# ValentinoGuerrini/Configurable-Hierarchical-Allreduce-Algorithms

Hardware: AMD Instinct MI355X
Metric: device-resident bucket-reduction GB/s (fp32); allreduce GB/s at 2/4/8 GPUs (higher is better)
Workload: dtype f32; 1 GPU; C2 bucket reduction: k=2 (m=1 incoming bucket), 64 MiB fp32 per bucket, device-resident, MPI_Reduce_local semantics; bucket_bytes=67108864, m=1, buffer_sets=16, parallelism=replicas, gate=untimed spin kernel ahead of the start event

## Files before the change

### include/chiara_user_op.hpp

```cpp
#pragma once

#include <hip/hip_runtime.h>

#include <cstddef>
#include <cstdint>
#include <type_traits>

#include "chiara.h"

namespace chr_user {

constexpr int kMaxIns = 16;
#ifndef CHR_USER_FOLD_U
#define CHR_USER_FOLD_U 4
#endif
constexpr int kU = CHR_USER_FOLD_U;

struct FoldArgs {
    void* out;
    const void* acc;
    const void* ins[kMaxIns];
    int m;
    size_t n;
    int running_first;
    int vec;
};

template <typename T>
struct FoldVec {
    static constexpr int kN = (sizeof(T) <= 16 && 16 % sizeof(T) == 0) ? int(16 / sizeof(T)) : 1;
    T e[kN];
};

typedef unsigned int tree_w4 __attribute__((ext_vector_type(4)));
typedef unsigned int tree_w2 __attribute__((ext_vector_type(2)));

#ifndef CHR_USER_GROUP_VEC
#define CHR_USER_GROUP_VEC 1
#endif
constexpr bool group_fold_pays(size_t s) { return s == 48; }
constexpr bool group_tree_pays(size_t s) { return s == 32; }
constexpr size_t gcd16(size_t s) {
    size_t g = 16;
    while (s % g) g >>= 1;
    return g;
}
template <typename T>
struct Grp {
    static constexpr size_t S = sizeof(T), G = S / gcd16(S) * 16;
    static constexpr int V = int(G / 16), E = int(G / S), kHeads = int(16 / gcd16(S));
    static constexpr bool kWide = 16 % S != 0;
    static constexpr bool kCan = kWide && V <= 8;
    static constexpr bool kFold = kCan && (CHR_USER_GROUP_VEC == 2 || (CHR_USER_GROUP_VEC == 1 && group_fold_pays(S)));
    static constexpr bool kTree =
        kCan && S % 4 == 0 && (CHR_USER_GROUP_VEC == 2 || (CHR_USER_GROUP_VEC == 1 && group_tree_pays(S)));
    static constexpr int kFoldU = !kFold ? 0 : 8 / V < kU ? 8 / V : kU;
};
template <int V> struct GrpW { tree_w4 w[V]; };
template <typename T> struct GrpE { T e[Grp<T>::E]; };
template <typename T> struct GrpPad { T t; unsigned char pad[(sizeof(T) + 3) / 4 * 4 - sizeof(T)]; };
template <typename T, typename OP>
__device__ __forceinline__ GrpW<Grp<T>::V> grp_map(const GrpW<Grp<T>::V>& a, const GrpW<Grp<T>::V>& b, OP op) {
    constexpr int V = Grp<T>::V, E = Grp<T>::E;
    using W = GrpW<V>;
    if constexpr (sizeof(T) % 4 == 0) {
        const GrpE<T> ae = __builtin_bit_cast(GrpE<T>, a), be = __builtin_bit_cast(GrpE<T>, b);
        GrpE<T> re;
#pragma unroll
        for (int e = 0; e < E; ++e) re.e[e] = op(ae.e[e], be.e[e]);
        return __builtin_bit_cast(W, re);
    } else {
        constexpr int S = (int)sizeof(T), NT = (S + 3) / 4, NW = 4 * V;
        struct Words { uint32_t w[NW]; };
        struct Elem { uint32_t w[NT]; };
        const Words aw = __builtin_bit_cast(Words, a), bw = __builtin_bit_cast(Words, b);
        Words rw = {};
        auto get = [](const Words& g, int o) {
            Elem t;
#pragma unroll
            for (int k = 0; k < NT; ++k) {
                const int q = o / 4 + k, sh = o % 4 * 8;
                uint32_t lo = g.w[q];
                if (sh) lo = (lo >> sh) | (q + 1 < NW ? g.w[q + 1] << (32 - sh) : 0u);
                t.w[k] = lo;
            }
            return __builtin_bit_cast(GrpPad<T>, t).t;
        };
#pragma unroll
        for (int e = 0; e < E; ++e) {
            GrpPad<T> p = {};
            p.t = op(get(aw, e * S), get(bw, e * S));
            const Elem t = __builtin_bit_cast(Elem, p);
#pragma unroll
            for (int k = 0; k < NT; ++k) {
                const int nb = S - 4 * k < 4 ? S - 4 * k : 4, o = e * S + 4 * k, q = o / 4, sh = o % 4 * 8;
                const uint32_t v = nb == 4 ? t.w[k] : t.w[k] & ((1u << (8 * nb)) - 1u);
                rw.w[q] |= v << sh;
                if (sh && sh + 8 * nb > 32) rw.w[q + 1] |= v >> (32 - sh);
            }
        }
        return __builtin_bit_cast(W, rw);
    }
}

inline bool congruent16(const void* p, const void* q) { return (((uintptr_t)p ^ (uintptr_t)q) & 15) == 0; }
template <typename T>
inline int group_head(const void* p, size_t n) {
    for (int h = 0; h < Grp<T>::kHeads; ++h)
        if ((((uintptr_t)p + (uintptr_t)h * sizeof(T)) & 15) == 0) return (size_t)h <= n ? h : -1;
    return -1;
}

template <typename T, typename F>
__device__ __forceinline__ void fold_groups(const FoldArgs& a) {
    constexpr int V = Grp<T>::V, E = Grp<T>::E, U = Grp<T>::kFoldU;
    using W = GrpW<V>;
    const F f{};
    const size_t tid = (size_t)blockIdx.x * blockDim.x + threadIdx.x;
    const size_t stride = (size_t)gridDim.x * blockDim.x;
    const size_t h = (size_t)a.vec - 1, ngrp = (a.n - h) / E, off = h * sizeof(T);
    const bool rf = a.running_first != 0;
    const W* accg = reinterpret_cast<const W*>(static_cast<const char*>(a.acc) + off);
    W* outg = reinterpret_cast<W*>(static_cast<char*>(a.out) + off);
    auto one = [&](T r, T x) { return f(rf ? r : x, rf ? x : r); };
    auto comb = [&](W& r, const W& x) { r = grp_map<T>(r, x, one); };
    const size_t chunk = (size_t)U * blockDim.x;
    const size_t nfull = ngrp / chunk;
    for (size_t c = blockIdx.x; c < nfull; c += gridDim.x) {
        const size_t base = c * chunk + threadIdx.x;
        W r[U];
#pragma unroll
        for (int u = 0; u < U; ++u) r[u] = accg[base + (size_t)u * blockDim.x];
        for (int j = 0; j < a.m; ++j) {
            const W* ing = reinterpret_cast<const W*>(static_cast<const char*>(a.ins[j]) + off);
            W x[U];
#pragma unroll
            for (int u = 0; u < U; ++u) x[u] = ing[base + (size_t)u * blockDim.x];
#pragma unroll
            for (int u = 0; u < U; ++u) comb(r[u], x[u]);
        }
#pragma unroll
        for (int u = 0; u < U; ++u) outg[base + (size_t)u * blockDim.x] = r[u];
    }
    for (size_t g = nfull * chunk + tid; g < ngrp; g += stride) {
        W r = accg[g];
        for (int j = 0; j < a.m; ++j)
            comb(r, reinterpret_cast<const W*>(static_cast<const char*>(a.ins[j]) + off)[g]);
        outg[g] = r;
    }
    const size_t tail0 = h + ngrp * E, extra = h + (a.n - tail0);
    for (size_t t = tid; t < extra; t += stride) {
        const size_t i = t < h ? t : tail0 + (t - h);
        T r = static_cast<const T*>(a.acc)[i];
        for (int j = 0; j < a.m; ++j) r = one(r, static_cast<const T*>(a.ins[j])[i]);
        static_cast<T*>(a.out)[i] = r;
    }
}

template <typename T, typename F>
__global__ void k_fold(FoldArgs a) {
    using V = FoldVec<T>;
    constexpr int kN = V::kN;
    const F f{};
    const size_t tid = (size_t)blockIdx.x * blockDim.x + threadIdx.x;
    const size_t stride = (size_t)gridDim.x * blockDim.x;
    if constexpr (Grp<T>::kFold) {
        if (a.vec) {
            fold_groups<T, F>(a);
            return;
        }
    }
    size_t done = 0;
    if (kN > 1 && a.vec) {
        const size_t nv = a.n / kN;
        const V* accv = static_cast<const V*>(a.acc);
        V* outv = static_cast<V*>(a.out);
        const size_t chunk = (size_t)kU * blockDim.x;
        const size_t nfull = nv / chunk;
        for (size_t c = blockIdx.x; c < nfull; c += gridDim.x) {
            const size_t base = c * chunk + threadIdx.x;
            V r[kU];
#pragma unroll
            for (int u = 0; u < kU; ++u) r[u] = accv[base + (size_t)u * blockDim.x];
            for (int j = 0; j < a.m; ++j) {
                const V* inv = static_cast<const V*>(a.ins[j]);
                V x[kU];
#pragma unroll
                for (int u = 0; u < kU; ++u) x[u] = inv[base + (size_t)u * blockDim.x];
#pragma unroll
                for (int u = 0; u < kU; ++u)
#pragma unroll
                    for (int e = 0; e < kN; ++e)
                        r[u].e[e] = a.running_first ? f(r[u].e[e], x[u].e[e]) : f(x[u].e[e], r[u].e[e]);
            }
#pragma unroll
            for (int u = 0; u < kU; ++u) outv[base + (size_t)u * blockDim.x] = r[u];
        }
        for (size_t v = nfull * chunk + tid; v < nv; v += stride) {
            V r = accv[v];
            for (int j = 0; j < a.m; ++j) {
                const V x = static_cast<const V*>(a.ins[j])[v];
#pragma unroll
                for (int e = 0; e < kN; ++e) r.e[e] = a.running_first ? f(r.e[e], x.e[e]) : f(x.e[e], r.e[e]);
            }
            outv[v] = r;
        }
        done = nv * kN;
    }
    for (size_t i = done + tid; i < a.n; i += stride) {
        T r = static_cast<const T*>(a.acc)[i];
        for (int j = 0; j < a.m; ++j) {
            const T x = static_cast<const T*>(a.ins[j])[i];
            r = a.running_first ? f(r, x) : f(x, r);
        }
        static_cast<T*>(a.out)[i] = r;
    }
}

template <typename T, typename F>
int launch_fold(void* out, const void* acc, const void* const* ins, int m, size_t n, int running_first,
                hipStream_t stream) {
    if (m < 0) return 1;
    const unsigned block = 256;
    auto aligned = [](const void* p) { return ((uintptr_t)p & 15) == 0; };
    bool vec = aligned(out) && aligned(acc);
    for (int j = 0; j < m; ++j) vec = vec && aligned(ins[j]);
    size_t lanes = vec ? (n / FoldVec<T>::kN + kU - 1) / kU + n % FoldVec<T>::kN : n;
    int head = -1;
    if constexpr (Grp<T>::kFold) {
        bool same = congruent16(out, acc);
        for (int j = 0; j < m; ++j) same = same && congruent16(out, ins[j]);
        if (same) head = group_head<T>(out, n);
        if (head >= 0)
            lanes = ((n - head) / Grp<T>::E + Grp<T>::kFoldU - 1) / Grp<T>::kFoldU + Grp<T>::kHeads + Grp<T>::E;
        else
            lanes = n;
    }
    const size_t blocks = (lanes + block - 1) / block;
    const unsigned grid = (unsigned)(blocks < 4096 ? (blocks ? blocks : 1) : 4096);
    int done = 0;
    const void* cur = acc;
    do {
        FoldArgs a{};
        a.out = out;
        a.acc = cur;
        a.m = m - done < kMaxIns ? m - done : kMaxIns;
        for (int j = 0; j < a.m; ++j) a.ins[j] = ins[done + j];
        a.n = n;
        a.running_first = running_first;
        a.vec = Grp<T>::kFold ? head + 1 : vec ? 1 : 0;
        hipLaunchKernelGGL((k_fold<T, F>), dim3(grid), dim3(block), 0, stream, a);
        if (hipGetLastError() != hipSuccess) return 1;
        done += a.m;
        cur = out;
    } while (done < m);
    return 0;
}

constexpr int kMaxLeaves = 8;
constexpr int kMaxTreesPerLaunch = 8;
constexpr int kTreeBlock = 64;
constexpr size_t kMaxLeafBytes = (size_t)1 << 37;
constexpr uint32_t kMaxElementwiseBlocks = 4096;

template <int NL>
constexpr int tree_u() {
    return NL <= 2 ? 4 : NL <= 4 ? 2 : 1;
}
template <typename T, int NL>
constexpr int tree_u_for() {
    if (!Grp<T>::kWide) return tree_u<NL>();
    if (!Grp<T>::kTree) return 0;
    return 8 / (NL * Grp<T>::V) < tree_u<NL>() ? 8 / (NL * Grp<T>::V) : tree_u<NL>();
}
#ifndef CHR_USER_TREE_WIDE_ELEMENTWISE
#define CHR_USER_TREE_WIDE_ELEMENTWISE 1
#endif
#ifndef CHR_USER_TREE_WG_PER_CU
#define CHR_USER_TREE_WG_PER_CU(NL) ((NL) <= 4 ? 12 : 16)
#endif

#ifndef CHR_USER_TREE_NT
#define CHR_USER_TREE_NT 1
#endif
#ifndef CHR_USER_TREE_XCD_RUN_KIB
#define CHR_USER_TREE_XCD_RUN_KIB 256
#endif

__device__ __forceinline__ tree_w4 tree_ld(const tree_w4* p) {
#if CHR_USER_TREE_NT
    return __builtin_nontemporal_load(p);
#else
    return *p;
#endif
}
__device__ __forceinline__ void tree_st(tree_w4* p, tree_w4 v) {
#if CHR_USER_TREE_NT
    __builtin_nontemporal_store(v, p);
#else
    *p = v;
#endif
}

template <int TRIP_BYTES>
__device__ __forceinline__ uint32_t tree_trip(uint32_t lb, uint32_t nblk) {
    constexpr uint32_t R = (uint32_t)CHR_USER_TREE_XCD_RUN_KIB * 1024u / TRIP_BYTES;
    if constexpr (R > 1) {
        constexpr uint32_t span = 8 * R;
        if (lb < nblk / span * span) {
            const uint32_t w = lb % span;
            return lb - w + (w % 8) * R + w / 8;
        }
    }
    return lb;
}

struct TreeSeg {
    void* out;
    const void* leaves[kMaxLeaves];
    size_t n;
    uint32_t comb;
    uint32_t swaps;
    uint32_t vec;
    uint32_t nblk;
};
struct TreeArgs {
    uint32_t block0[kMaxTreesPerLaunch];
    TreeSeg seg[kMaxTreesPerLaunch];
};

template <typename T, bool ARITH = std::is_arithmetic<T>::value, size_t SZ = sizeof(T)>
struct TreeSlot { using S = T; };
template <typename T> struct TreeSlot<T, false, 4> { using S = uint32_t; };
template <typename T> struct TreeSlot<T, false, 8> { using S = tree_w2; };
template <typename T> struct TreeSlot<T, false, 16> { using S = tree_w4; };

template <typename T, typename F>
struct TreeApVec {
    using S = tree_w4;
    __device__ __forceinline__ static S ap(S in, S run) {
        using V = FoldVec<T>;
        const V x = __builtin_bit_cast(V, in);
        V r = __builtin_bit_cast(V, run);
        const F f{};
#pragma unroll
        for (int e = 0; e < V::kN; ++e) r.e[e] = f(x.e[e], r.e[e]);
        return __builtin_bit_cast(S, r);
    }
};
template <typename T, typename F>
struct TreeApGrp {
    using S = GrpW<Grp<T>::V>;
    __device__ __forceinline__ static S ap(const S& in, const S& run) {
        return grp_map<T>(in, run, [](const T& x, const T& r) { return F{}(x, r); });
    }
};
template <typename T, typename F>
struct TreeApOne {
    using S = typename TreeSlot<T>::S;
    __device__ __forceinline__ static S ap(S in, S run) {
        return __builtin_bit_cast(S, F{}(__builtin_bit_cast(T, in), __builtin_bit_cast(T, run)));
    }
};

template <typename A, int NL, int W, bool WIDE = false>
__device__ __forceinline__ void tree_eval(const typename A::S (&x)[NL][W], typename A::S (&r)[W], uint32_t comb,
                                          uint32_t swaps) {
    using S = typename A::S;
#pragma unroll
    for (int w = 0; w < W; ++w) {
        S s0 = x[0][w], s1 = s0, s2 = s0, s3 = s0;
        int d = 1, ci = 0;
#pragma unroll
        for (int j = 1; j < NL; ++j) {
            const S v = x[j][w];
            if constexpr (WIDE) {
                if (d == 1) s1 = v;
                else if (j > 1 && d == 2) s2 = v;
                else if (j > 2) s3 = v;
            } else {
                if (d == 1) s1 = v;
                else if (d == 2) s2 = v;
                else s3 = v;
            }
            ++d;
            for (int c = (int)((comb >> (2 * j)) & 3u); c > 0; --c, ++ci) {
                const bool sw = (swaps >> ci) & 1u;
                if constexpr (WIDE) {
                    if (j == 1 || d == 2) {
                        if (sw) s0 = A::ap(s0, s1);
                        else s0 = A::ap(s1, s0);
                    } else if (j == 2 || d == 3) {
                        if (sw) s1 = A::ap(s1, s2);
                        else s1 = A::ap(s2, s1);
                    } else {
                        if (sw) s2 = A::ap(s2, s3);
                        else s2 = A::ap(s3, s2);
                    }
                } else {
                    if (d == 2) s0 = A::ap(sw ? s0 : s1, sw ? s1 : s0);
                    else if (d == 3) s1 = A::ap(sw ? s1 : s2, sw ? s2 : s1);
                    else s2 = A::ap(sw ? s2 : s3, sw ? s3 : s2);
                }
                --d;
            }
        }
        r[w] = s0;
    }
}

template <typename T, typename F, int NL>
__device__ __forceinline__ void tree_one(const TreeSeg& g, size_t i) {
    using A = TreeApOne<T, F>;
    using S = typename A::S;
    S x[NL][1], r[1];
#pragma unroll
    for (int j = 0; j < NL; ++j) x[j][0] = __builtin_bit_cast(S, static_cast<const T*>(g.leaves[j])[i]);
    tree_eval<A, NL, 1, Grp<T>::kWide>(x, r, g.comb, g.swaps);
    static_cast<T*>(g.out)[i] = __builtin_bit_cast(T, r[0]);
}

template <typename T, typename F, int NL, int U, int BL>
__global__ __launch_bounds__(BL) void k_tree(TreeArgs a) {
    using V = FoldVec<T>;
    constexpr int kN = V::kN;
    const uint32_t b = blockIdx.x;
    int s = 0;
#pragma unroll
    for (int j = 1; j < kMaxTreesPerLaunch; ++j)
        if (b >= a.block0[j]) s = j;
    const TreeSeg& g = a.seg[s];
    const uint32_t nblk = g.nblk;
    if (b - a.block0[s] >= nblk) return;
    constexpr int kTripBytes = U == 0 ? BL * (int)sizeof(T) : BL * U * 16 * (Grp<T>::kWide ? Grp<T>::V : 1);
    const uint32_t lb = tree_trip<kTripBytes>(b - a.block0[s], nblk);
    const size_t n = g.n;
    if constexpr (Grp<T>::kTree && U > 0) if (g.vec) {
        using A = TreeApGrp<T, F>;
        using W = typename A::S;
        constexpr int E = Grp<T>::E;
        const size_t h = g.vec - 1, ngrp = (n - h) / E, nfull = ngrp / ((size_t)BL * U), off = h * sizeof(T);
        const uint32_t comb = g.comb, swaps = g.swaps;
        W* const out = reinterpret_cast<W*>(static_cast<char*>(g.out) + off);
        const W* lv[NL];
#pragma unroll
        for (int j = 0; j < NL; ++j) lv[j] = reinterpret_cast<const W*>(static_cast<const char*>(g.leaves[j]) + off);
        if (lb < nfull) {
            const size_t base = (size_t)lb * BL * U + threadIdx.x;
            W x[NL][U], r[U];
#pragma unroll
            for (int j = 0; j < NL; ++j)
#pragma unroll
                for (int u = 0; u < U; ++u)
#pragma unroll
                    for (int v = 0; v < Grp<T>::V; ++v) x[j][u].w[v] = tree_ld(&lv[j][base + (size_t)u * BL].w[v]);
            __builtin_amdgcn_sched_barrier(0);
            tree_eval<A, NL, U, true>(x, r, comb, swaps);
#pragma unroll
            for (int u = 0; u < U; ++u)
#pragma unroll
                for (int v = 0; v < Grp<T>::V; ++v) tree_st(&out[base + (size_t)u * BL].w[v], r[u].w[v]);
        }
        if (lb == nfull) {
            for (size_t i = nfull * BL * U + threadIdx.x; i < ngrp; i += BL) {
                W x[NL][1], r[1];
#pragma unroll
                for (int j = 0; j < NL; ++j) x[j][0] = lv[j][i];
                tree_eval<A, NL, 1, true>(x, r, comb, swaps);
                out[i] = r[0];
            }
        }
        if (lb == 0) {
            const size_t tail0 = h + ngrp * E, t = threadIdx.x;
            const size_t i = t < h ? t : tail0 + (t - h);
            if (i < n) tree_one<T, F, NL>(g, i);
        }
        return;
    }
    if constexpr (sizeof(V) == 16) if (g.vec) {
        using A = TreeApVec<T, F>;
        const size_t nvec = n / kN, nfull = nvec / ((size_t)BL * U);
        const uint32_t comb = g.comb, swaps = g.swaps;
        tree_w4* const out = static_cast<tree_w4*>(g.out);
        const tree_w4* lv[NL];
#pragma unroll
        for (int j = 0; j < NL; ++j) lv[j] = static_cast<const tree_w4*>(g.leaves[j]);
        if (lb < nfull) {
            const size_t base = (size_t)lb * BL * U + threadIdx.x;
            tree_w4 x[NL][U], r[U];
#pragma unroll
            for (int j = 0; j < NL; ++j)
#pragma unroll
                for (int u = 0; u < U; ++u) x[j][u] = tree_ld(&lv[j][base + (size_t)u * BL]);
            __builtin_amdgcn_sched_barrier(0);
            tree_eval<A, NL, U>(x, r, comb, swaps);
#pragma unroll
            for (int u = 0; u < U; ++u) tree_st(&out[base + (size_t)u * BL], r[u]);
        }
        if (lb == nfull) {
            for (size_t i = nfull * BL * U + threadIdx.x; i < nvec; i += BL) {
                tree_w4 x[NL][1], r[1];
#pragma unroll
                for (int j = 0; j < NL; ++j) x[j][0] = lv[j][i];
                tree_eval<A, NL, 1>(x, r, comb, swaps);
                out[i] = r[0];
            }
        }
        if (lb == 0 && nvec * kN + threadIdx.x < n) tree_one<T, F, NL>(g, nvec * kN + threadIdx.x);
        return;
    }
    for (size_t i = (size_t)lb * BL + threadIdx.x; i < n; i += (size_t)nblk * BL) tree_one<T, F, NL>(g, i);
}

inline unsigned tree_lds_bytes(int wg_per_cu) {
    static const struct Lds {
        int cu = 0, blk = 0;
        Lds() {
            int dev = 0;
            if (hipGetDevice(&dev) != hipSuccess ||
                hipDeviceGetAttribute(&cu, hipDeviceAttributeMaxSharedMemoryPerMultiprocessor, dev) != hipSuccess ||
                hipDeviceGetAttribute(&blk, hipDeviceAttributeMaxSharedMemoryPerBlock, dev) != hipSuccess)
                cu = blk = 0;
        }
    } lds;
    if (wg_per_cu <= 0 || lds.cu <= 0 || lds.blk <= 0) return 0;
    const unsigned bytes = ((unsigned)lds.cu / (unsigned)wg_per_cu) & ~255u;
    return bytes > (unsigned)lds.blk ? (unsigned)lds.blk & ~255u : bytes;
}

template <typename T, typename F, int NL>
void launch_tree_nl(const chr_user_tree* const* trees, int ntrees, int wg_per_cu, hipStream_t stream) {
    constexpr int U = tree_u_for<T, NL>(), BL = kTreeBlock;
    constexpr bool kVecT = sizeof(FoldVec<T>) == 16;
    constexpr bool kGrpT = Grp<T>::kTree && U > 0;
    static_assert(!kGrpT || Grp<T>::kHeads + Grp<T>::E <= BL, "head and tail elements: one lane each");
    const unsigned lds = tree_lds_bytes(wg_per_cu > 0 ? wg_per_cu : CHR_USER_TREE_WG_PER_CU(NL));
    auto aligned = [](const void* p) { return ((uintptr_t)p & 15) == 0; };
    for (int t0 = 0; t0 < ntrees; t0 += kMaxTreesPerLaunch) {
        TreeArgs a{};
        uint32_t grid = 0;
        for (int k = 0; k < kMaxTreesPerLaunch; ++k) {
            if (t0 + k >= ntrees) {
                a.block0[k] = ~0u;
                continue;
            }
            const chr_user_tree& t = *trees[t0 + k];
            TreeSeg& g = a.seg[k];
            g.out = t.out;
            bool vec = kVecT && aligned(t.out);
            int ci = 0;
            for (int j = 0; j < NL; ++j) {
                g.leaves[j] = t.leaves[j];
                vec = vec && aligned(t.leaves[j]);
                g.comb |= (uint32_t)(t.comb[j] & 3u) << (2 * j);
                for (int c = 0; c < t.comb[j] && ci < 8; ++c, ++ci) g.swaps |= (uint32_t)(t.swaps[ci] & 1u) << ci;
            }
            g.n = t.n;
            g.vec = vec ? 1 : 0;
            const size_t per = vec ? (size_t)BL * U * FoldVec<T>::kN : (size_t)BL;
            size_t want = (t.n + per - 1) / per;
            if constexpr (kGrpT) {
                bool same = true;
                for (int j = 0; j < NL; ++j) same = same && congruent16(t.out, t.leaves[j]);
                const int head = same ? group_head<T>(t.out, t.n) : -1;
                if (head >= 0) {
                    vec = true;
                    g.vec = 1u + (uint32_t)head;
                    const size_t ngrp = (t.n - head) / Grp<T>::E, trip = (size_t)BL * U;
                    want = ngrp < trip ? 1 : (ngrp + trip - 1) / trip;
                }
            }
            g.nblk = (uint32_t)(vec || want < kMaxElementwiseBlocks ? want : kMaxElementwiseBlocks);
            a.block0[k] = grid;
            grid += (g.nblk + 7u) & ~7u;
        }
        hipLaunchKernelGGL((k_tree<T, F, NL, U, BL>), dim3(grid), dim3(BL), lds, stream, a);
    }
}

template <typename T, typename F>
int launch_tree(const chr_user_tree* trees, int ntrees, int wg_per_cu, hipStream_t stream) {
    if (ntrees < 0 || (ntrees && !trees)) return 1;
    for (int t = 0; t < ntrees; ++t) {
        const chr_user_tree& tr = trees[t];
        if (tr.nleaves < 2 || tr.nleaves > kMaxLeaves || tr.n == 0 || tr.n > kMaxLeafBytes / sizeof(T) ||
            !tr.out)
            return 1;
        int d = 0;
        for (int j = 0; j < tr.nleaves; ++j) {
            if (!tr.leaves[j] || ++d > 4 || tr.comb[j] > 3 || tr.comb[j] >= d) return 1;
            d -= tr.comb[j];
        }
        if (d != 1) return 1;
        if (Grp<T>::kTree && !CHR_USER_TREE_WIDE_ELEMENTWISE && tr.nleaves * Grp<T>::V > 8) return 1;
    }
    const chr_user_tree* grp[64];
    for (int nl = 2; nl <= kMaxLeaves; ++nl) {
        int k = 0;
        auto flush = [&] {
            if (k == 0) return;
            switch (nl) {
            case 2: launch_tree_nl<T, F, 2>(grp, k, wg_per_cu, stream); break;
            case 3: launch_tree_nl<T, F, 3>(grp, k, wg_per_cu, stream); break;
            case 4: launch_tree_nl<T, F, 4>(grp, k, wg_per_cu, stream); break;
            case 5: launch_tree_nl<T, F, 5>(grp, k, wg_per_cu, stream); break;
            case 6: launch_tree_nl<T, F, 6>(grp, k, wg_per_cu, stream); break;
            case 7: launch_tree_nl<T, F, 7>(grp, k, wg_per_cu, stream); break;
            default: launch_tree_nl<T, F, 8>(grp, k, wg_per_cu, stream); break;
            }
            k = 0;
        };
        for (int t = 0; t < ntrees; ++t)
            if (trees[t].nleaves == nl) {
                grp[k++] = &trees[t];
                if (k == 64) flush();
            }
        flush();
    }
    return 0;
}

}

#define CHR_DEFINE_USER_TREE(name, T, F)                                                                             \
    extern "C" int name(const chr_user_tree* trees, int ntrees, chr_dtype, int wg_per_cu, hipStream_t stream,        \
                        void*) {                                                                                     \
        return chr_user::launch_tree<T, F>(trees, ntrees, wg_per_cu, stream);                                        \
    }

#define CHR_DEFINE_USER_TREE_FOR(name, T, F, DTYPE)                                                                   \
    extern "C" int name(const chr_user_tree* trees, int ntrees, chr_dtype dt, int wg_per_cu, hipStream_t stream,     \
                        void*) {                                                                                     \
        if (dt != (DTYPE)) return 1;                                                                                 \
        return chr_user::launch_tree<T, F>(trees, ntrees, wg_per_cu, stream);                                        \
    }

#define CHR_DEFINE_USER_OP(name, T, F)                                                                               \
    extern "C" int name(void* out, const void* acc, const void* const* ins, int m, size_t n, chr_dtype,             \
                        int running_first, hipStream_t stream, void*) {                                           \
        return chr_user::launch_fold<T, F>(out, acc, ins, m, n, running_first, stream);                           \
    }

#define CHR_DEFINE_USER_OP_FOR(name, T, F, DTYPE)                                                                     \
    extern "C" int name(void* out, const void* acc, const void* const* ins, int m, size_t n, chr_dtype dt,          \
                        int running_first, hipStream_t stream, void*) {                                           \
        if (dt != (DTYPE)) return 1;                                                                                 \
        return chr_user::launch_fold<T, F>(out, acc, ins, m, n, running_first, stream);                           \
    }
```

Measured before the change: 6744 GB/s.

## Add streaming fold kernel with XCD-aware block mapping for large buckets

Adds a specialized streaming path for the fold (reduce_local) kernel on large, aligned, non-wide types. Each 64-thread block handles a fixed tile with U-way unroll and nontemporal loads and stores. Block indices are remapped so consecutive runs of memory stay on one XCD, kernel arguments are pinned to SGPRs, and LDS is reserved to cap workgroups per CU. The tree path also gets a plain (cached) first load and an optional SGPR pin. The aim is to get closer to HBM streaming bandwidth for the 64 MiB m=1 case, at the cost of extra template instantiations and a size-threshold dispatch.

```diff
diff --git a/include/chiara_user_op.hpp b/include/chiara_user_op.hpp
--- a/include/chiara_user_op.hpp
+++ b/include/chiara_user_op.hpp
@@ -24,6 +24,7 @@
     size_t n;
     int running_first;
     int vec;
+    int stream;
 };
 
 template <typename T>
@@ -157,10 +158,119 @@
     }
 }
 
+#ifndef CHR_USER_FOLD_STREAM_MIN_BYTES
+#define CHR_USER_FOLD_STREAM_MIN_BYTES ((size_t)40 << 20)
+#endif
+constexpr int kMaxStreamIns = 8;
+constexpr int kStreamBlock = 64;
+constexpr int kStreamWgPerCu = 12;
+constexpr int stream_u(int m) { return m == 1 ? 4 : m <= 3 ? 2 : 1; }
+constexpr int stream_run_kib(int m) { return m <= 3 ? 256 : 512; }
+
+template <typename P>
+__device__ __forceinline__ void pin_sgpr(P p) {
+    asm volatile("" ::"s"(p));
+}
+
+template <int TRIP_BYTES, int RUN_KIB>
+__device__ __forceinline__ uint32_t xcd_run_trip(uint32_t lb, uint32_t nblk) {
+    constexpr uint32_t R = (uint32_t)RUN_KIB * 1024u / TRIP_BYTES;
+    if constexpr (R > 1) {
+        constexpr uint32_t span = 8 * R;
+        if (lb < nblk / span * span) {
+            const uint32_t w = lb % span;
+            return lb - w + (w % 8) * R + w / 8;
+        }
+    }
+    return lb;
+}
+
+inline unsigned tree_lds_bytes(int wg_per_cu);
+
+template <typename T, typename F, int M>
+__device__ __forceinline__ void fold_stream(const FoldArgs& a) {
+    using V = FoldVec<T>;
+    constexpr int kN = V::kN, U = stream_u(M), BL = kStreamBlock;
+    static_assert(sizeof(V) == 16 && kN <= BL, "FoldVec's sizes only");
+    const F f{};
+    tree_w4* const out = static_cast<tree_w4*>(a.out);
+    const tree_w4* const accp = static_cast<const tree_w4*>(a.acc);
+    const tree_w4* ins[M];
+#pragma unroll
+    for (int j = 0; j < M; ++j) ins[j] = static_cast<const tree_w4*>(a.ins[j]);
+    const size_t n = a.n;
+    const int rf = a.running_first;
+    pin_sgpr(out);
+    pin_sgpr(accp);
+    pin_sgpr(n);
+    pin_sgpr(rf);
+#pragma unroll
+    for (int j = 0; j < M; ++j) pin_sgpr(ins[j]);
+    const size_t nv = n / kN, nfull = nv / ((size_t)BL * U);
+    const size_t lb = xcd_run_trip<BL * U * 16, stream_run_kib(M)>(blockIdx.x, gridDim.x);
+    auto comb = [&](tree_w4& r, tree_w4 x) {
+        const V p = __builtin_bit_cast(V, rf ? r : x), q = __builtin_bit_cast(V, rf ? x : r);
+        V o;
+#pragma unroll
+        for (int e = 0; e < kN; ++e) o.e[e] = f(p.e[e], q.e[e]);
+        r = __builtin_bit_cast(tree_w4, o);
+    };
+    if (lb < nfull) {
+        const size_t base = lb * BL * U + threadIdx.x;
+        tree_w4 r[U], x[M][U];
+        r[0] = accp[base];
+#pragma unroll
+        for (int u = 1; u < U; ++u) r[u] = __builtin_nontemporal_load(&accp[base + (size_t)u * BL]);
+#pragma unroll
+        for (int j = 0; j < M; ++j)
+#pragma unroll
+            for (int u = 0; u < U; ++u) x[j][u] = __builtin_nontemporal_load(&ins[j][base + (size_t)u * BL]);
+        __builtin_amdgcn_sched_barrier(0);
+#pragma unroll
+        for (int j = 0; j < M; ++j)
+#pragma unroll
+            for (int u = 0; u < U; ++u) comb(r[u], x[j][u]);
+#pragma unroll
+        for (int u = 0; u < U; ++u) __builtin_nontemporal_store(r[u], &out[base + (size_t)u * BL]);
+    } else if (lb == nfull) {
+        for (size_t i = nfull * BL * U + threadIdx.x; i < nv; i += BL) {
+            tree_w4 r = accp[i], x[M];
+#pragma unroll
+            for (int j = 0; j < M; ++j) x[j] = ins[j][i];
+#pragma unroll
+            for (int j = 0; j < M; ++j) comb(r, x[j]);
+            out[i] = r;
+        }
+        const size_t i = nv * kN + threadIdx.x;
+        if (i < n) {
+            T r = static_cast<const T*>(a.acc)[i], x[M];
+#pragma unroll
+            for (int j = 0; j < M; ++j) x[j] = static_cast<const T*>(a.ins[j])[i];
+#pragma unroll
+            for (int j = 0; j < M; ++j) r = rf ? f(r, x[j]) : f(x[j], r);
+            static_cast<T*>(a.out)[i] = r;
+        }
+    }
+}
+
 template <typename T, typename F>
 __global__ void k_fold(FoldArgs a) {
     using V = FoldVec<T>;
     constexpr int kN = V::kN;
+    if constexpr (!Grp<T>::kWide) {
+        if (a.stream) {
+            switch (a.m) {
+            case 1: return fold_stream<T, F, 1>(a);
+            case 2: return fold_stream<T, F, 2>(a);
+            case 3: return fold_stream<T, F, 3>(a);
+            case 4: return fold_stream<T, F, 4>(a);
+            case 5: return fold_stream<T, F, 5>(a);
+            case 6: return fold_stream<T, F, 6>(a);
+            case 7: return fold_stream<T, F, 7>(a);
+            default: return fold_stream<T, F, 8>(a);
+            }
+        }
+    }
     const F f{};
     const size_t tid = (size_t)blockIdx.x * blockDim.x + threadIdx.x;
     const size_t stride = (size_t)gridDim.x * blockDim.x;
@@ -238,18 +348,33 @@
     }
     const size_t blocks = (lanes + block - 1) / block;
     const unsigned grid = (unsigned)(blocks < 4096 ? (blocks ? blocks : 1) : 4096);
+    auto stream_grid = [&](int k) -> size_t {
+        if (Grp<T>::kWide || !vec || k < 1 || k > kMaxStreamIns || n == 0) return 0;
+        constexpr size_t kN = FoldVec<T>::kN;
+        const size_t per = (size_t)kStreamBlock * stream_u(k) * kN;
+        const size_t g = n / per + (n % per ? 1 : 0);
+        if (g >= ((size_t)1 << 31)) return 0;
+        return (size_t)(k + 2) * n * sizeof(T) >= (size_t)(CHR_USER_FOLD_STREAM_MIN_BYTES) ? g : 0;
+    };
+    const int per_launch = stream_grid(m < kMaxStreamIns ? m : kMaxStreamIns) ? kMaxStreamIns : kMaxIns;
     int done = 0;
     const void* cur = acc;
     do {
         FoldArgs a{};
         a.out = out;
         a.acc = cur;
-        a.m = m - done < kMaxIns ? m - done : kMaxIns;
+        a.m = m - done < per_launch ? m - done : per_launch;
         for (int j = 0; j < a.m; ++j) a.ins[j] = ins[done + j];
         a.n = n;
         a.running_first = running_first;
         a.vec = Grp<T>::kFold ? head + 1 : vec ? 1 : 0;
-        hipLaunchKernelGGL((k_fold<T, F>), dim3(grid), dim3(block), 0, stream, a);
+        if (const size_t sg = stream_grid(a.m)) {
+            a.stream = 1;
+            hipLaunchKernelGGL((k_fold<T, F>), dim3((unsigned)sg), dim3(kStreamBlock), tree_lds_bytes(kStreamWgPerCu),
+                               stream, a);
+        } else {
+            hipLaunchKernelGGL((k_fold<T, F>), dim3(grid), dim3(block), 0, stream, a);
+        }
         if (hipGetLastError() != hipSuccess) return 1;
         done += a.m;
         cur = out;
@@ -286,6 +411,12 @@
 #ifndef CHR_USER_TREE_XCD_RUN_KIB
 #define CHR_USER_TREE_XCD_RUN_KIB 256
 #endif
+#ifndef CHR_USER_TREE_ACC0
+#define CHR_USER_TREE_ACC0 1
+#endif
+#ifndef CHR_USER_TREE_PIN
+#define CHR_USER_TREE_PIN 0
+#endif
 
 __device__ __forceinline__ tree_w4 tree_ld(const tree_w4* p) {
 #if CHR_USER_TREE_NT
@@ -304,15 +435,7 @@
 
 template <int TRIP_BYTES>
 __device__ __forceinline__ uint32_t tree_trip(uint32_t lb, uint32_t nblk) {
-    constexpr uint32_t R = (uint32_t)CHR_USER_TREE_XCD_RUN_KIB * 1024u / TRIP_BYTES;
-    if constexpr (R > 1) {
-        constexpr uint32_t span = 8 * R;
-        if (lb < nblk / span * span) {
-            const uint32_t w = lb % span;
-            return lb - w + (w % 8) * R + w / 8;
-        }
-    }
-    return lb;
+    return xcd_run_trip<TRIP_BYTES, CHR_USER_TREE_XCD_RUN_KIB>(lb, nblk);
 }
 
 struct TreeSeg {
@@ -485,13 +608,22 @@
         const tree_w4* lv[NL];
 #pragma unroll
         for (int j = 0; j < NL; ++j) lv[j] = static_cast<const tree_w4*>(g.leaves[j]);
+#if CHR_USER_TREE_PIN
+        pin_sgpr(out);
+        pin_sgpr(n);
+#pragma unroll
+        for (int j = 0; j < NL; ++j) pin_sgpr(lv[j]);
+#endif
         if (lb < nfull) {
             const size_t base = (size_t)lb * BL * U + threadIdx.x;
             tree_w4 x[NL][U], r[U];
 #pragma unroll
             for (int j = 0; j < NL; ++j)
 #pragma unroll
-                for (int u = 0; u < U; ++u) x[j][u] = tree_ld(&lv[j][base + (size_t)u * BL]);
+                for (int u = 0; u < U; ++u) {
+                    if (CHR_USER_TREE_ACC0 && j == 0 && u == 0) x[j][u] = lv[j][base];
+                    else x[j][u] = tree_ld(&lv[j][base + (size_t)u * BL]);
+                }
             __builtin_amdgcn_sched_barrier(0);
             tree_eval<A, NL, U>(x, r, comb, swaps);
 #pragma unroll
```

Result: no change. 6741 GB/s (-0.0%).
